# syl051088/DynaAlign

Measured on AMD Instinct MI355X. Metric: sequence-pairs/sec (MinHash k=4 n_hash=500; NW BLOSUM62) at 1/2/4/8 MI355X, higher is better.
Workload: dtype u32

## Files before the change

dynaalign_amd/csrc/minhash_kernels.hip:

```cpp
#include "da_common.hpp"

#include <algorithm>
#include <atomic>
#include <mutex>
#include <vector>
#include <type_traits>

namespace da {
namespace {

__device__ __forceinline__ uint32_t rotl32(uint32_t v, int r) {
  return __builtin_rotateleft32(v, r);
}
__device__ __forceinline__ uint32_t mm3_scramble(uint32_t w) {
  w *= 0xcc9e2d51u;
  w = rotl32(w, 15);
  w *= 0x1b873593u;
  return w;
}
__device__ __forceinline__ uint32_t mm3_mix(uint32_t h, uint32_t kk) {
  h ^= kk;
  return rotl32(h, 13) * 5u + 0xe6546b64u;
}
__device__ __forceinline__ uint32_t mm3_final(uint32_t h, uint32_t len) {
// ... 1442 lines not shown
      uint32_t hi[8] = {0, 0, 0, 0, 0, 0, 0, 0};
      for (int k = 0; k < nhi; ++k) {
        const uint32_t b = blk[rows * W + ((int64_t)k * rows + row) * groups + (col >> 3)];
#pragma unroll
        for (int e = 0; e < 8; ++e) hi[e] |= ((b >> e) & 1u) << (8 + k);
      }
      st[q].x = ((lo.x & 255u) | hi[0]) | ((((lo.x >> 8) & 255u) | hi[1]) << 16);
      st[q].y = (((lo.x >> 16) & 255u) | hi[2]) | (((lo.x >> 24) | hi[3]) << 16);
      st[q].z = ((lo.y & 255u) | hi[4]) | ((((lo.y >> 8) & 255u) | hi[5]) << 16);
      st[q].w = (((lo.y >> 16) & 255u) | hi[6]) | (((lo.y >> 24) | hi[7]) << 16);
    }
  }
  if (!IS_NW)
    for (int e = tid; e < tab_entries; e += 256) tab[e] = (double)e / (double)n_hash;
#pragma unroll
  for (int q = 0; q < 8; ++q) *reinterpret_cast<uint4 *>(er_lds + (row0 + 16 * q) * ER_STRIDE + unit * 16) = st[q];
  __syncthreads();
  auto widen = [&](uint32_t x) -> double {
    if (!IS_NW) return tab_entries ? tab[x] : (double)x / (double)n_hash;
    const uint32_t ln = x & 255u;
    if (ln == 0) return __longlong_as_double(0xFFF8000000000000ULL);
    return (double)(x >> 8) / (double)ln;
  };
  er_store_tile(er_lds, widen, out, ld, I0, J0, tx, ty);
}
static bool finalize_rows_ok(const ShardGeom &geom, const void *d_g, int64_t ld_g, const double *d_out, int64_t ld, bool packed) {
  return geom.tile == 128 && geom.n >= 256 && (ld & 1) == 0 && (reinterpret_cast<uintptr_t>(d_out) & 15) == 0 &&
         (reinterpret_cast<uintptr_t>(d_g) & 15) == 0 && (packed || (ld_g & 7) == 0);
}

template <int FT>
__device__ __forceinline__ void store_tile_u16(const uint16_t (&t)[FT][FT + 2], uint16_t *__restrict__ out, int64_t ld, int n, int i0, int j0) {
  constexpr int RS = 256 / FT;
  const int tx = threadIdx.x & (FT - 1), ty = threadIdx.x / FT;
  const int j = j0 + tx;
  uint16_t *o = out + (int64_t)i0 * ld + j;
  for (int r = ty; r < FT; r += RS) {
    const int i = i0 + r;
    if (i < n && j < n && j >= i) o[(int64_t)r * ld] = t[r][tx];
  }
  const int im = i0 + tx;
  uint16_t *om = out + (int64_t)j0 * ld + im;
  for (int r = ty; r < FT; r += RS) {
    const int jm = j0 + r;
    if (im < n && jm < n && jm > im) om[(int64_t)r * ld] = t[tx][r];
  }
}
template <bool IS_NW, bool U16 = false>
__global__ __launch_bounds__(256) void k_finalize_sharded(const uint16_t *__restrict__ G, int64_t ld_g, ShardGeom geom,
                                                          int n_hash, void *__restrict__ out_v, int64_t ld, int TB,
                                                          int64_t ntiles, int64_t per_xcd, int skip_fast) {
  double *out = static_cast<double *>(out_v);
  constexpr int FT = 64, TABLE = 2048;
  __shared__ uint16_t t[FT][FT + 2];
  __shared__ double ratio[IS_NW ? 1 : TABLE];
  const int n = (int)geom.n;
  const TileId tt = skip_fast ? leftover_tile64(blockIdx.x, n, TB) : decode_tile_xcd(blockIdx.x, per_xcd, ntiles, TB);
  if (!tt.valid) return;
  const int i0 = tt.ti * FT, j0 = tt.tj * FT;
  const int tx = threadIdx.x & 63, ty = threadIdx.x >> 6;
  const bool use_table = !IS_NW && n_hash < TABLE;
  if (use_table)
    for (int c = threadIdx.x; c <= n_hash; c += 256) ratio[c] = (double)c / (double)n_hash;
  auto widen = [&](uint32_t v) -> double {
    if (!IS_NW) return use_table ? ratio[v] : (double)v / (double)n_hash;
    const uint32_t ln = v & 255u;
    if (ln == 0) return __longlong_as_double(0xFFF8000000000000ULL);
    return (double)(v >> 8) / (double)ln;
  };
  const int tile = geom.tile;
  const int tr = i0 / tile;
  const int q = tr / geom.world, owner = tr - q * geom.world;
  const bool front = q <= geom.Q - 1 - q;
  const int64_t lrow0 = (int64_t)owner * geom.rows + (int64_t)(front ? q : geom.Q - 1 - q) * tile + (i0 - tr * tile);
  const int64_t coff = front ? -(int64_t)tr * tile : shard_back(geom.W, geom.n);
  const uint16_t *src = G + lrow0 * ld_g + coff + j0 + tx;
  const int j = j0 + tx;
  for (int r = ty; r < FT; r += 4) {
    const int i = i0 + r;
    if (i < n && j < n && j >= i) t[r][tx] = src[(int64_t)r * ld_g];
  }
  __syncthreads();
  if (U16) store_tile_u16<64>(t, static_cast<uint16_t *>(out_v), ld, n, i0, j0);
  else store_tile_f64<64>(t, widen, out, ld, n, i0, j0);
}

template <bool F64, bool IS_NW, int FT>
__global__ __launch_bounds__(256) void k_expand_unique(const uint16_t *__restrict__ D, int64_t ld_d, const int32_t *__restrict__ uidx,
                                                       int n, int n_hash, void *__restrict__ out_v, int64_t ld, int TB,
                                                       int64_t ntiles, int64_t per_xcd, int skip_fast, TableRows trows) {
  __shared__ uint16_t t[FT][FT + 2];
  __shared__ int32_t ur[FT], uc[FT];
  const TileId tt = skip_fast ? leftover_tile64(blockIdx.x, n, TB) : decode_tile_xcd(blockIdx.x, per_xcd, ntiles, TB);
  if (!tt.valid) return;
  const int i0 = tt.ti * FT, j0 = tt.tj * FT;
  constexpr int RS = 256 / FT;
  const int tx = threadIdx.x & (FT - 1), ty = threadIdx.x / FT;
  for (int q = threadIdx.x; q < 2 * FT; q += 256) {
    if (q < FT) ur[q] = (i0 + q < n) ? uidx[i0 + q] : 0;
    else uc[q - FT] = (j0 + q - FT < n) ? uidx[j0 + q - FT] : 0;
  }
  __syncthreads();
  auto widen = [&](uint32_t v) -> double {
    if (!IS_NW) return (double)v / (double)n_hash;
    const uint32_t ln = v & 255u;
    if (ln == 0) return __longlong_as_double(0xFFF8000000000000ULL);
    return (double)(v >> 8) / (double)ln;
  };
  const int j = j0 + tx;
  const int32_t cj = uc[tx];
  for (int r = ty; r < FT; r += RS) {
    const int i = i0 + r;
    if (i < n && j < n && j >= i) t[r][tx] = D[table_row(ur[r], trows) * ld_d + cj];
  }
  __syncthreads();
  if (F64) {
    store_tile_f64<FT>(t, widen, reinterpret_cast<double *>(out_v), ld, n, i0, j0);
  } else {
    uint16_t *out = reinterpret_cast<uint16_t *>(out_v);
    uint16_t *o = out + (int64_t)i0 * ld + j;
    for (int r = ty; r < FT; r += RS) {
      const int i = i0 + r;
      if (i < n && j < n && j >= i) o[(int64_t)r * ld] = t[r][tx];
    }
    const int im = i0 + tx;
    uint16_t *om = out + (int64_t)j0 * ld + im;
    for (int r = ty; r < FT; r += RS) {
      const int jm = j0 + r;
      if (im < n && jm < n && jm > im) om[(int64_t)r * ld] = t[tx][r];
    }
  }
}

constexpr int GC_THREADS = 1024;
__global__ __launch_bounds__(GC_THREADS) void k_gather_columns(const uint16_t *__restrict__ D, int64_t ld_d, const int32_t *__restrict__ uidx,
                                                               const int32_t *__restrict__ ufirst, int n, int U, uint16_t *__restrict__ F,
                                                               int64_t ld_f, TableRows trows, int from_first_tile, int row_begin) {
  extern __shared__ __attribute__((aligned(16))) uint16_t gc_row[];
  const int units = (int)(ld_d >> 3);
  uint4 pre[8];
#define GC_FETCH(row)                                                                                   \
  {                                                                                                     \
    const uint4 *src_ = reinterpret_cast<const uint4 *>(D + table_row((row), trows) * ld_d);            \
    _Pragma("unroll") for (int q = 0; q < 8; ++q) {                                                     \
      const int u = (int)threadIdx.x + q * GC_THREADS;                                                  \
      pre[q] = u < units ? src_[u] : make_uint4(0, 0, 0, 0);                                            \
    }                                                                                                   \
  }
  int r = row_begin + (int)blockIdx.x;
  if (r < U) GC_FETCH(r)
  const int2 *u2 = reinterpret_cast<const int2 *>(uidx);
  const int j2_end = n >> 1;
  for (; r < U; r += gridDim.x) {
    __syncthreads();
    uint4 *dst = reinterpret_cast<uint4 *>(gc_row);
#pragma unroll
    for (int q = 0; q < 8; ++q) {
      const int u = (int)threadIdx.x + q * GC_THREADS;
      if (u < units) dst[u] = pre[q];
    }
    __syncthreads();
    if (r + (int)gridDim.x < U) GC_FETCH(r + (int)gridDim.x)
    const int j_begin = ((ufirst[r] >> 7) + (from_first_tile ? 0 : 1)) << 7;
    uint32_t *frow = reinterpret_cast<uint32_t *>(F + (int64_t)r * ld_f);
    for (int j2 = (j_begin >> 1) + threadIdx.x; j2 < j2_end; j2 += GC_THREADS) {
      const int2 c = u2[j2];
      __builtin_nontemporal_store((uint32_t)gc_row[c.x] | ((uint32_t)gc_row[c.y] << 16), frow + j2);
    }
    if ((n & 1) && threadIdx.x == 0 && n - 1 >= j_begin) F[(int64_t)r * ld_f + n - 1] = gc_row[uidx[n - 1]];
  }
#undef GC_FETCH
}

template <bool IS_NW>
__global__ __launch_bounds__(256, 4) void k_expand_rows(const uint16_t *__restrict__ F, int64_t ld_f, const int32_t *__restrict__ uidx,
                                                        int n, int n_hash, int tab_stride, int tab_entries, double *__restrict__ out,
                                                        int64_t ld, int T128, int64_t ntiles, int64_t per_xcd, int64_t tile_begin) {
  extern __shared__ __attribute__((aligned(16))) unsigned char er_lds[];
  double *tab = reinterpret_cast<double *>(er_lds + 128 * ER_STRIDE);
  const int64_t L = tile_begin + (int64_t)(blockIdx.x & 7) * per_xcd + (blockIdx.x >> 3);
  if (L >= ntiles || L >= tile_begin + (int64_t)((blockIdx.x & 7) + 1) * per_xcd) return;
  const TileId tt = decode_tile(L, T128, T128, true);
  if (!tt.valid || !expand_fast_takes(tt.ti, tt.tj, n, ld, out)) return;
  const int tid = threadIdx.x, wave = tid >> 6, lane = tid & 63;
  const int tx = ((wave & 1) << 3) + (lane & 7), ty = ((wave >> 1) << 3) + (lane >> 3);
  const int64_t I0 = (int64_t)tt.ti * 128, J0 = (int64_t)tt.tj * 128;
  uint4 st[8];
#pragma unroll
  for (int q = 0; q < 8; ++q) {
    const int row = (tid >> 4) + 16 * q;
    st[q] = *(reinterpret_cast<const uint4 *>(F + (int64_t)uidx[I0 + row] * ld_f + J0) + (tid & 15));
  }
  if (IS_NW) {
    for (int e = tid; e < tab_entries; e += 256) {
      const int mt = e / tab_stride, ln = e - mt * tab_stride;
      tab[e] = ln == 0 ? __longlong_as_double(0xFFF8000000000000ULL) : (double)mt / (double)ln;
    }
  } else {
    for (int e = tid; e < tab_entries; e += 256) tab[e] = (double)e / (double)n_hash;
  }
#pragma unroll
  for (int q = 0; q < 8; ++q)
    *reinterpret_cast<uint4 *>(er_lds + ((tid >> 4) + 16 * q) * ER_STRIDE + (tid & 15) * 16) = st[q];
  __syncthreads();
  auto widen = [&](uint32_t x) -> double {
    if (IS_NW) return tab[(x >> 8) * (uint32_t)tab_stride + (x & 255u)];
    return tab[x];
  };
  er_store_tile(er_lds, widen, out, ld, I0, J0, tx, ty);
}

constexpr int ES_THREADS = 1024, ES_COPIES = 4, ES_BATCH = 16;
__global__ __launch_bounds__(256) void k_es_zero(uint32_t *__restrict__ w, int words) {
  const int i = blockIdx.x * 256 + threadIdx.x;
  if (i < words) w[i] = 0u;
}
__global__ __launch_bounds__(256) void k_es_count(const int32_t *__restrict__ uidx, int n, int U, int Z, uint32_t *__restrict__ cnt) {
  const int i = blockIdx.x * 256 + threadIdx.x;
  if (i < n) atomicAdd(&cnt[(i / Z) * U + uidx[i]], 1u);
}
__device__ __forceinline__ uint64_t es_scan_load(const uint32_t *__restrict__ cnt, int K, int i) {
  const uint32_t c = i < K ? cnt[i] : 0u;
  return (uint64_t)c | ((uint64_t)((c + ES_COPIES - 1) / ES_COPIES) << 32);
}
__global__ __launch_bounds__(1024) void k_es_scan_sums(const uint32_t *__restrict__ cnt, int K, uint64_t *__restrict__ bsum) {
  __shared__ uint64_t wsum[16];
  uint64_t x = es_scan_load(cnt, K, blockIdx.x * 1024 + threadIdx.x);
#pragma unroll
  for (int d = 32; d >= 1; d >>= 1) x += __shfl_xor(x, d, 64);
  if ((threadIdx.x & 63) == 0) wsum[threadIdx.x >> 6] = x;
  __syncthreads();
  if (threadIdx.x == 0) { uint64_t t = 0; for (int w = 0; w < 16; ++w) t += wsum[w]; bsum[blockIdx.x] = t; }
}
__global__ __launch_bounds__(1024) void k_es_scan_offsets(uint64_t *__restrict__ bsum, int nblocks) {
  __shared__ uint64_t wsum[16];
  __shared__ uint64_t carry_s;
  const int tid = threadIdx.x, lane = tid & 63, wave = tid >> 6;
  if (tid == 0) carry_s = 0;
  __syncthreads();
  for (int base = 0; base < nblocks; base += 1024) {
    const int i = base + tid;
    const uint64_t v = i < nblocks ? bsum[i] : 0;
    uint64_t x = v;
#pragma unroll
    for (int d = 1; d < 64; d <<= 1) {
      const uint64_t y = __shfl_up(x, d, 64);
      if (lane >= d) x += y;
    }
    if (lane == 63) wsum[wave] = x;
    __syncthreads();
    uint64_t woff = 0;
    for (int w = 0; w < wave; ++w) woff += wsum[w];
    const uint64_t carry = carry_s;
    if (i < nblocks) bsum[i] = carry + woff + x - v;
    __syncthreads();
    if (tid == 1023) carry_s = carry + woff + x;
    __syncthreads();
  }
  if (tid == 0) bsum[nblocks] = carry_s;
}
__global__ __launch_bounds__(1024) void k_es_scan_apply(const uint32_t *__restrict__ cnt, int K, const uint64_t *__restrict__ bsum,
                                                        uint32_t *__restrict__ cstart, uint32_t *__restrict__ zstart) {
  __shared__ uint64_t wsum[16];
  const int tid = threadIdx.x, lane = tid & 63, wave = tid >> 6;
  const int i = blockIdx.x * 1024 + tid;
  const uint64_t v = es_scan_load(cnt, K, i);
  uint64_t x = v;
#pragma unroll
  for (int d = 1; d < 64; d <<= 1) {
    const uint64_t y = __shfl_up(x, d, 64);
    if (lane >= d) x += y;
  }
  if (lane == 63) wsum[wave] = x;
  __syncthreads();
  uint64_t woff = bsum[blockIdx.x];
  for (int w = 0; w < wave; ++w) woff += wsum[w];
  const uint64_t e = woff + x - v;
  if (i < K) { cstart[i] = (uint32_t)e; zstart[i] = (uint32_t)(e >> 32); }
  if (blockIdx.x == gridDim.x - 1 && tid == 0) { const uint64_t t = bsum[gridDim.x]; cstart[K] = (uint32_t)t; zstart[K] = (uint32_t)(t >> 32); }
}
__global__ __launch_bounds__(256) void k_es_fill(const int32_t *__restrict__ uidx, int n, int U, int Z, int K, const uint32_t *__restrict__ cstart,
                                                 const uint32_t *__restrict__ zstart, uint32_t *__restrict__ cursor, int32_t *__restrict__ cpos,
                                                 int2 *__restrict__ items) {
  const int i = blockIdx.x * 256 + threadIdx.x;
  if (i < n) {
    const int key = (i / Z) * U + uidx[i];
    cpos[cstart[key] + atomicAdd(&cursor[key], 1u)] = i;
  }
  if (i < K) {
    const uint32_t first = zstart[i], cnt = zstart[i + 1] - first;
    for (uint32_t q = 0; q < cnt; ++q) items[first + q] = make_int2(i % U, (int)(q * ES_COPIES));
  }
}
__device__ __forceinline__ double es_ratio(uint32_t c, double dn, double rcp) {
  const double dc = (double)c, q0 = __dmul_rn(dc, rcp), e = __fma_rn(-q0, dn, dc);
  return __fma_rn(e, rcp, q0);
}
__global__ __launch_bounds__(256) void k_es_ratio_check(int n_hash, double *__restrict__ out) {
  const int c = blockIdx.x * 256 + threadIdx.x;
  const double dn = (double)n_hash, rcp = 1.0 / dn;
  if (c <= n_hash) out[c] = es_ratio((uint32_t)c, dn, rcp);
}
enum { ES_U16 = 0, ES_U16_PK = 1, ES_PK = 2 };
#ifdef ES_STEAL_COUNT
__device__ unsigned es_steal[64][ES_ZONES][2];
#endif
template <int FMT, int NQ>
__global__ __launch_bounds__(ES_THREADS, 8)
void k_expand_stream(const uint16_t *__restrict__ D, int64_t ld_d, const int32_t *__restrict__ uidx,
                                                              const uint32_t *__restrict__ cstart, const int32_t *__restrict__ cpos,
                                                              const int2 *__restrict__ items, const uint32_t *__restrict__ zstart, int U, int zones,
                                                              int row_end, int n, int n_hash, double *__restrict__ out, int64_t ld,
                                                              uint32_t *ticket, int max_batch) {
  extern __shared__ __attribute__((aligned(16))) unsigned char es_lds[];
#ifdef ES_PRIO
  __builtin_amdgcn_s_setprio(ES_PRIO);
#endif
  constexpr bool PACKED = FMT != ES_U16;
  uint16_t *row = reinterpret_cast<uint16_t *>(es_lds);
  unsigned char *row_lo = es_lds, *row_hi = row_lo + ld_d;
  const int tid = threadIdx.x;
  const double dn = (double)n_hash, rcp = 1.0 / dn;
  auto count_of = [&](int c) -> uint32_t {
    if (!PACKED) return row[c];
    return (uint32_t)row_lo[c] | ((((uint32_t)row_hi[c >> 3] >> (c & 7)) & 1u) << 8);
  };
  const int64_t row_bytes = FMT == ES_PK ? pk_row_bytes(ld_d) : 2 * ld_d;
  const int units = (int)(row_bytes >> 4);
  uint4 pre[NQ];
#define ES_FETCH(r_)                                                                                    \
  {                                                                                                     \
    const uint4 *src_ = reinterpret_cast<const uint4 *>(reinterpret_cast<const unsigned char *>(D) + (int64_t)(r_) * row_bytes); \
    _Pragma("unroll") for (int q = 0; q < NQ; ++q) {                                                    \
      const int u = tid + q * ES_THREADS;                                                               \
      pre[q] = u < units ? src_[u] : make_uint4(0, 0, 0, 0);                                            \
    }                                                                                                   \
  }
  __shared__ int s_next, s_end, s_zone;
  unsigned home;
  asm volatile("s_getreg_b32 %0, hwreg(HW_REG_XCC_ID)" : "=s"(home));
  home = (home & 7u) % (unsigned)zones;
  const uint32_t home_z0 = zstart[home * U], home_lim = zstart[home * U + row_end] - home_z0,
                 home_all = zstart[home * U + U] - home_z0;
  const uint32_t share = max(1u, gridDim.x / (unsigned)zones);
  auto take = [&]() {
    int tz = -1, tk = 0, te = 0;
    for (int t = 0; t < zones && tz < 0; ++t) {
      const int z = (int)((home + (unsigned)t) % (unsigned)zones);
      const uint32_t z0 = t ? zstart[z * U] : home_z0, lim = t ? zstart[z * U + row_end] - z0 : home_lim,
                     all = t ? zstart[z * U + U] - z0 : home_all;
      uint32_t cur = __hip_atomic_load(&ticket[z], __ATOMIC_RELAXED, __HIP_MEMORY_SCOPE_AGENT);
      while (cur < lim) {
        const uint32_t b = min(min((uint32_t)max_batch, lim - cur), max(1u, (all - cur) / share));
        const uint32_t old = atomicCAS(&ticket[z], cur, cur + b);
#ifdef ES_STEAL_COUNT
        if (old == cur) atomicAdd(&es_steal[min(63, (row_end + 1023) >> 10)][home][t ? 1 : 0], b);
#endif
        if (old == cur) { tz = z; tk = (int)(z0 + cur); te = tk + (int)b; break; }
        cur = old;
      }
    }
    s_zone = tz; s_next = tk; s_end = te;
  };
  if (tid == 0) take();
  __syncthreads();
  int z = __builtin_amdgcn_readfirstlane(s_zone), k = __builtin_amdgcn_readfirstlane(s_next), k_end = __builtin_amdgcn_readfirstlane(s_end);
  int2 it = z >= 0 ? items[k] : make_int2(0, 0);
  if (z >= 0) ES_FETCH(it.x)
  const int2 *u2 = reinterpret_cast<const int2 *>(uidx);
  const int j2_end = n >> 1;
  while (z >= 0) {
    __syncthreads();
    const bool more = k + 1 < k_end;
    if (tid == 0 && !more) take();
    uint4 *dst = reinterpret_cast<uint4 *>(row);
#pragma unroll
    for (int q = 0; q < NQ; ++q) {
      const int u = tid + q * ES_THREADS;
      if (u >= units) continue;
      if (FMT != ES_U16_PK) { dst[u] = pre[q]; continue; }
      const uint4 v = pre[q];
      uint2 lo;
      lo.x = __builtin_amdgcn_perm(v.y, v.x, 0x06040200u);
      lo.y = __builtin_amdgcn_perm(v.w, v.z, 0x06040200u);
      *reinterpret_cast<uint2 *>(row_lo + 8 * u) = lo;
      row_hi[u] = (unsigned char)(((v.x >> 8) & 1u) | ((v.x >> 23) & 2u) | ((v.y >> 6) & 4u) | ((v.y >> 21) & 8u) | ((v.z >> 4) & 16u) |
                                  ((v.z >> 19) & 32u) | ((v.w >> 2) & 64u) | ((v.w >> 17) & 128u));
    }
    __syncthreads();
    const int key = z * U + it.x;
    const uint32_t c0 = cstart[key] + (uint32_t)it.y, c_end = cstart[key + 1];
    const int ncop = (int)min((uint32_t)ES_COPIES, c_end - c0);
    double *orow[ES_COPIES];
#pragma unroll
    for (int q = 0; q < ES_COPIES; ++q) orow[q] = out + (int64_t)cpos[c0 + (uint32_t)min(q, ncop - 1)] * ld;
    const int zn = more ? z : __builtin_amdgcn_readfirstlane(s_zone), kn = more ? k + 1 : __builtin_amdgcn_readfirstlane(s_next);
    if (!more) k_end = __builtin_amdgcn_readfirstlane(s_end);
    int2 itn = make_int2(0, 0);
    if (zn >= 0) { itn = items[kn]; ES_FETCH(itn.x) }
#pragma unroll 4
    for (int j2 = tid; j2 < j2_end; j2 += ES_THREADS) {
      const int2 c = u2[j2];
      const double v0 = es_ratio(count_of(c.x), dn, rcp), v1 = es_ratio(count_of(c.y), dn, rcp);
      nt_store2(orow[0] + 2 * j2, v0, v1);
      if (ncop > 1) nt_store2(orow[1] + 2 * j2, v0, v1);
      if (ncop > 2) nt_store2(orow[2] + 2 * j2, v0, v1);
      if (ncop > 3) nt_store2(orow[3] + 2 * j2, v0, v1);
    }
    if ((n & 1) && tid == 0) {
      const double v = es_ratio(count_of(uidx[n - 1]), dn, rcp);
      for (int q = 0; q < ncop; ++q) orow[q][n - 1] = v;
    }
    it = itn;
    z = zn;
    k = kn;
  }
#undef ES_FETCH
}

bool expand_stream_ok(int64_t n, int64_t U, int n_hash, const void *d_out, int64_t ld) {
  return n >= 2 && n <= 0x7fffffffLL && U >= 1 && U <= 65536 && n_hash >= 1 && n_hash <= 2047 && (ld & 1) == 0 &&
         (reinterpret_cast<uintptr_t>(d_out) & 15) == 0;
}
extern "C" int da_debug_ratio_check(int n_hash, double *d_out, void *stream) {
  if (n_hash < 1 || !d_out) return fail(DA_ERR_BAD_ARG, "ratio check: bad arguments");
  hipLaunchKernelGGL(k_es_ratio_check, dim3((unsigned)(n_hash / 256 + 1)), dim3(256), 0, static_cast<hipStream_t>(stream), n_hash, d_out);
  DA_HIP_TRY(hipGetLastError());
  return DA_OK;
}
#ifdef ES_STEAL_COUNT
extern "C" int da_debug_expand_steals(unsigned *out, int reset) {
  static const unsigned zero[64 * ES_ZONES * 2] = {};
  DA_HIP_TRY(hipDeviceSynchronize());
  if (out) DA_HIP_TRY(hipMemcpyFromSymbol(out, HIP_SYMBOL(es_steal), sizeof(zero)));
  if (reset) DA_HIP_TRY(hipMemcpyToSymbol(HIP_SYMBOL(es_steal), zero, sizeof(zero)));
  return DA_OK;
}
#endif
bool expand_stream_packed(int n_hash) { return n_hash <= 511; }
static int es_zones() { return config().mh_expand_zones == 1 ? 1 : ES_ZONES; }
int expand_stream_zones() { return es_zones(); }
struct EsLists { uint32_t *cnt, *cursor, *ticket, *cstart, *zstart; int32_t *cpos; int2 *items; uint64_t *bsum; int zones, Z, K; size_t bytes; };
static EsLists es_layout(void *d_scratch, int64_t n, int64_t U, int zones) {
  uint32_t *w = static_cast<uint32_t *>(d_scratch);
  EsLists L;
  const int64_t K = (int64_t)zones * U;
  L.zones = zones; L.Z = (int)zone_rows(n, zones); L.K = (int)K;
  L.cnt = w; L.cursor = w + K; L.ticket = w + 2 * K; L.cstart = L.ticket + ES_ZONES; L.zstart = L.cstart + (K + 1);
  L.cpos = reinterpret_cast<int32_t *>(L.zstart + (K + 1));
  L.items = reinterpret_cast<int2 *>((reinterpret_cast<uintptr_t>(L.cpos + n) + 15) & ~(uintptr_t)15);
  L.bsum = reinterpret_cast<uint64_t *>(L.items + (std::min(n, K) + n / ES_COPIES + 2));
  L.bytes = (size_t)(reinterpret_cast<unsigned char *>(L.bsum + (ceil_div(K, 1024) + 1)) - static_cast<unsigned char *>(d_scratch));
  return L;
}
size_t expand_stream_scratch_bytes(int64_t n, int64_t U) {
  return es_layout(nullptr, n, U, ES_ZONES).bytes + 16;
}
static int es_lists(const int32_t *d_uidx, int64_t n, int64_t U, void *d_scratch, int zones, hipStream_t stream) {
  const EsLists L = es_layout(d_scratch, n, U, zones);
  const int zero_words = 2 * L.K + ES_ZONES;
  hipLaunchKernelGGL(k_es_zero, dim3((unsigned)ceil_div(zero_words, 256)), dim3(256), 0, stream, L.cnt, zero_words);
  const unsigned nblk = (unsigned)ceil_div(L.K, 1024);
  hipLaunchKernelGGL(k_es_count, dim3((unsigned)ceil_div(n, 256)), dim3(256), 0, stream, d_uidx, (int)n, (int)U, L.Z, L.cnt);
  hipLaunchKernelGGL(k_es_scan_sums, dim3(nblk), dim3(1024), 0, stream, L.cnt, L.K, L.bsum);
  hipLaunchKernelGGL(k_es_scan_offsets, dim3(1), dim3(1024), 0, stream, L.bsum, (int)nblk);
  hipLaunchKernelGGL(k_es_scan_apply, dim3(nblk), dim3(1024), 0, stream, L.cnt, L.K, L.bsum, L.cstart, L.zstart);
  hipLaunchKernelGGL(k_es_fill, dim3((unsigned)ceil_div(std::max<int64_t>(n, L.K), 256)), dim3(256), 0, stream, d_uidx, (int)n, (int)U, L.Z, L.K,
                     L.cstart, L.zstart, L.cursor, L.cpos, L.items);
  DA_HIP_TRY(hipGetLastError());
  return DA_OK;
}
int launch_expand_stream_lists(const int32_t *d_uidx, int64_t n, int64_t U, void *d_scratch, hipStream_t stream) {
  return es_lists(d_uidx, n, U, d_scratch, es_zones(), stream);
}
extern "C" int da_debug_expand_lists(const int32_t *d_uidx, int64_t n, int64_t U, int zones, void *d_scratch, size_t scratch_bytes, int64_t *offsets_out,
                                     int *zones_out, void *stream) {
  if (zones == 0) zones = es_zones();
  if (n < 1 || n > 0x7fffffffLL || U < 1 || U > 65536 || U > n || (zones != 1 && zones != ES_ZONES) || !offsets_out)
    return fail(DA_ERR_BAD_ARG, "expand lists: bad arguments");
  const EsLists L = es_layout(d_scratch, n, U, zones);
  const unsigned char *b = static_cast<const unsigned char *>(d_scratch);
  offsets_out[0] = reinterpret_cast<const unsigned char *>(L.cstart) - b; offsets_out[1] = reinterpret_cast<const unsigned char *>(L.zstart) - b;
  offsets_out[2] = reinterpret_cast<const unsigned char *>(L.cpos) - b; offsets_out[3] = reinterpret_cast<const unsigned char *>(L.items) - b;
  offsets_out[4] = (int64_t)expand_stream_scratch_bytes(n, U); offsets_out[5] = L.Z;
  if (zones_out) *zones_out = zones;
  if (!d_scratch) return DA_OK;
  if (!d_uidx || scratch_bytes < (size_t)offsets_out[4] || (reinterpret_cast<uintptr_t>(d_scratch) & 15)) return fail(DA_ERR_BAD_ARG, "expand lists: bad scratch");
  return es_lists(d_uidx, n, U, d_scratch, zones, static_cast<hipStream_t>(stream));
}
static int es_launch(const uint16_t *d_D, int64_t ld_d, const int32_t *d_colids, int64_t n_cols, const EsLists &L, int64_t n_rows, int64_t U,
                     int64_t row_end, int n_hash, double *d_out, int64_t ld, hipStream_t stream, bool pk);
int launch_expand_stream_rows(const uint16_t *d_D, int64_t ld_d, const int32_t *d_uidx, int64_t n, int64_t U, int n_hash, double *d_out, int64_t ld,
                              void *d_scratch, int64_t row_end, hipStream_t stream, bool pk) {
  if (!expand_stream_ok(n, U, n_hash, d_out, ld) || (ld_d & (pk ? 127 : 7)) || ld_d > 65536 || (reinterpret_cast<uintptr_t>(d_D) & 15) ||
      (pk && !expand_stream_packed(n_hash)))
    return fail(DA_ERR_UNSUPPORTED, "row expansion: shape not covered");
  if (row_end > U) row_end = U;
  if (row_end <= 0) return DA_OK;
  return es_launch(d_D, ld_d, d_uidx, n, es_layout(d_scratch, n, U, es_zones()), n, U, row_end, n_hash, d_out, ld, stream, pk);
}
static int es_launch(const uint16_t *d_D, int64_t ld_d, const int32_t *d_uidx, int64_t n, const EsLists &L, int64_t n_rows, int64_t U,
                     int64_t row_end, int n_hash, double *d_out, int64_t ld, hipStream_t stream, bool pk) {
  static std::atomic<int> es_cus;
  static std::atomic<uint64_t> es_attr_done;
  int dev = 0;
  DA_HIP_TRY(hipGetDevice(&dev));
  if (!((es_attr_done.load() >> (dev & 63)) & 1u)) {
    hipDeviceProp_t prop;
    DA_HIP_TRY(hipGetDeviceProperties(&prop, dev));
#define DA_ES_ATTR(P, Q) DA_HIP_TRY(hipFuncSetAttribute(reinterpret_cast<const void *>(k_expand_stream<P, Q>), hipFuncAttributeMaxDynamicSharedMemorySize, 65536 * 2))
    DA_ES_ATTR(ES_U16, 2); DA_ES_ATTR(ES_U16, 4); DA_ES_ATTR(ES_U16, 6); DA_ES_ATTR(ES_U16, 8);
    DA_ES_ATTR(ES_U16_PK, 2); DA_ES_ATTR(ES_U16_PK, 4); DA_ES_ATTR(ES_U16_PK, 6); DA_ES_ATTR(ES_U16_PK, 8);
    DA_ES_ATTR(ES_PK, 2); DA_ES_ATTR(ES_PK, 4); DA_ES_ATTR(ES_PK, 6); DA_ES_ATTR(ES_PK, 8);
#undef DA_ES_ATTR
    es_cus.store(prop.multiProcessorCount > 0 ? prop.multiProcessorCount : 256);
    es_attr_done.fetch_or(1ull << (dev & 63));
  }
  const bool packed = pk || expand_stream_packed(n_hash);
  size_t lds = packed ? (size_t)pk_row_bytes(ld_d) : (size_t)ld_d * 2;
  lds = std::max<size_t>(lds, 82 * 1024);
  int64_t grid = (int64_t)es_cus.load();
  grid = std::min<int64_t>(grid, std::min<int64_t>(n_rows, L.K) + n_rows / ES_COPIES + 1);
#define DA_ES(P, Q) hipLaunchKernelGGL((k_expand_stream<P, Q>), dim3((unsigned)grid), dim3(ES_THREADS), lds, stream, d_D, ld_d, d_uidx, L.cstart, L.cpos, L.items, \
                                       L.zstart, (int)U, L.zones, (int)row_end, (int)n, n_hash, d_out, ld, L.ticket, ES_BATCH * ES_ZONES / L.zones)
  const int64_t nq = ceil_div((pk ? pk_row_bytes(ld_d) : 2 * ld_d) >> 4, ES_THREADS);
#define DA_ES_NQ(F) do { if (nq <= 2) DA_ES(F, 2); else if (nq <= 4) DA_ES(F, 4); else if (nq <= 6) DA_ES(F, 6); else DA_ES(F, 8); } while (0)
  if (pk) DA_ES_NQ(ES_PK);
  else if (packed) DA_ES_NQ(ES_U16_PK);
  else DA_ES_NQ(ES_U16);
#undef DA_ES_NQ
#undef DA_ES
  DA_HIP_TRY(hipGetLastError());
  return DA_OK;
}
int launch_expand_stream(const uint16_t *d_D, int64_t ld_d, const int32_t *d_uidx, int64_t n, int64_t U, int n_hash, double *d_out, int64_t ld,
                         void *d_scratch, hipStream_t stream, hipEvent_t after_lists, bool pk) {
  if (!expand_stream_ok(n, U, n_hash, d_out, ld)) return fail(DA_ERR_UNSUPPORTED, "row expansion: shape not covered");
  int rc = launch_expand_stream_lists(d_uidx, n, U, d_scratch, stream);
  if (rc != DA_OK) return rc;
  if (after_lists) DA_HIP_TRY(hipEventRecord(after_lists, stream));
  return launch_expand_stream_rows(d_D, ld_d, d_uidx, n, U, n_hash, d_out, ld, d_scratch, U, stream, pk);
}

bool expand_stream_rect_ok(int64_t m, int64_t n, int64_t U_x, int64_t U_y, int n_hash, const void *d_out, int64_t ld) {
  return m >= 1 && m <= 0x7ffffff0LL && n >= 1 && n <= 0x7ffffff0LL && U_x >= 1 && U_x <= m && U_y >= 1 && U_y <= 65536 && n_hash >= 1 &&
         n_hash <= 2047 && (ld & 1) == 0 && (reinterpret_cast<uintptr_t>(d_out) & 15) == 0;
}
int launch_expand_stream_rect(const uint16_t *d_D, int64_t ld_d, const int32_t *d_uidx_x, int64_t m, int64_t U_x, const int32_t *d_uidx_y, int64_t n,
                              int64_t U_y, int n_hash, double *d_out, int64_t ld, void *d_scratch, hipStream_t stream, hipEvent_t after_lists) {
  if (!expand_stream_rect_ok(m, n, U_x, U_y, n_hash, d_out, ld) || ld_d < U_y || (ld_d & 7) || ld_d > 65536 || (reinterpret_cast<uintptr_t>(d_D) & 15))
    return fail(DA_ERR_UNSUPPORTED, "rectangular row expansion: shape not covered");
  int rc = launch_expand_stream_lists(d_uidx_x, m, U_x, d_scratch, stream);
  if (rc != DA_OK) return rc;
  if (after_lists) DA_HIP_TRY(hipEventRecord(after_lists, stream));
  return es_launch(d_D, ld_d, d_uidx_y, n, es_layout(d_scratch, m, U_x, es_zones()), m, U_x, U_x, n_hash, d_out, ld, stream, false);
}

__global__ __launch_bounds__(256) void k_fill_sig_rows(uint32_t *__restrict__ sig, int64_t ld_sig, int64_t m, int64_t m_pad, int n_hash) {
  const int64_t r = m + blockIdx.x;
  if (r >= m_pad) return;
  const uint32_t *src = sig + ((r - m) % m) * ld_sig;
  for (int h = threadIdx.x; h < n_hash; h += 256) sig[r * ld_sig + h] = src[h];
}
int launch_fill_sig_rows(uint32_t *d_sig, int64_t ld_sig, int64_t m, int64_t m_pad, int n_hash, hipStream_t stream) {
  if (m_pad <= m || m <= 0) return DA_OK;
  hipLaunchKernelGGL(k_fill_sig_rows, dim3((unsigned)(m_pad - m)), dim3(256), 0, stream, d_sig, ld_sig, m, m_pad, n_hash);
  DA_HIP_TRY(hipGetLastError());
  return DA_OK;
}

size_t expand_rows_workspace_bytes(int64_t n, int64_t U, int kind, bool is_nw, int n_hash, int nw_max_len) {
  if (kind != DA_OUT_F64 || n < 256 || U > 65536 || U < 1) return 0;
  if (is_nw ? (nw_max_len < 1 || (int64_t)(nw_max_len + 1) * (2 * nw_max_len + 1) > 2048) : (n_hash < 1 || n_hash + 1 > 2048)) return 0;
  return (size_t)U * (size_t)(ceil_div(n, 8) * 8) * 2;
}

int launch_gather_columns(const uint16_t *d_D, int64_t ld_d, const int32_t *d_uidx, const int32_t *d_ufirst, int64_t n, int64_t U,
                          uint16_t *d_F, int64_t ld_f, bool from_first_tile, hipStream_t stream, int table_world, int64_t table_rows_local,
                          int64_t row_begin, int64_t row_end) {
  if (row_end < 0 || row_end > U) row_end = U;
  if (row_begin < 0) row_begin = 0;
  if (U >= 1 && row_begin >= row_end) return DA_OK;
  if (U < 1 || U > 65536 || (ld_d & 7) || ld_d > 65536 || (reinterpret_cast<uintptr_t>(d_D) & 15) || (ld_f & 1))
    return fail(DA_ERR_UNSUPPORTED, "column gather: at most 65536 unique strings, 16-byte aligned table rows");
  const TableRows trows{table_world, table_rows_local};
  const size_t row_bytes = (size_t)ld_d * 2;
  static std::atomic<int> gc_cus;
  static std::atomic<uint64_t> gc_attr_done;
  int dev = 0;
  DA_HIP_TRY(hipGetDevice(&dev));
  if (!((gc_attr_done.load() >> (dev & 63)) & 1u)) {
    hipDeviceProp_t prop;
    DA_HIP_TRY(hipGetDeviceProperties(&prop, dev));
    DA_HIP_TRY(hipFuncSetAttribute(reinterpret_cast<const void *>(k_gather_columns), hipFuncAttributeMaxDynamicSharedMemorySize, 65536 * 2));
    gc_cus.store(prop.multiProcessorCount > 0 ? prop.multiProcessorCount : 256);
    gc_attr_done.fetch_or(1ull << (dev & 63));
  }
  const int gc_wg = row_bytes <= 40 * 1024 ? 2 : 1;
  const int64_t gc_grid = std::min<int64_t>(row_end - row_begin, (int64_t)gc_cus.load() * gc_wg);
  hipLaunchKernelGGL(k_gather_columns, dim3((unsigned)gc_grid), dim3(GC_THREADS), row_bytes, stream, d_D, ld_d, d_uidx, d_ufirst, (int)n,
                     (int)row_end, d_F, ld_f, trows, from_first_tile ? 1 : 0, (int)row_begin);
  DA_HIP_TRY(hipGetLastError());
  return DA_OK;
}

int launch_expand_rows(const uint16_t *d_F, int64_t ld_f, const int32_t *d_uidx, int64_t n, bool is_nw, int n_hash, int nw_max_len,
                       double *d_out, int64_t ld, int64_t band_begin, int64_t band_end, hipStream_t stream) {
  const int T128 = (int)ceil_div(n, 128);
  if (band_end < 0) band_end = mh_sym_bands(n);
  const int64_t t0 = mh_sym_band_prefix(n, band_begin), t1 = mh_sym_band_prefix(n, band_end);
  if (t1 <= t0) return DA_OK;
  const int64_t px = ceil_div(t1 - t0, 8);
  const int stride = is_nw ? 2 * nw_max_len + 1 : 1;
  const int entries = is_nw ? (nw_max_len + 1) * stride : n_hash + 1;
  const size_t lds = 128 * ER_STRIDE + (size_t)entries * 8;
  if (is_nw) hipLaunchKernelGGL(k_expand_rows<true>, dim3((unsigned)(px * 8)), dim3(256), lds, stream, d_F, ld_f, d_uidx, (int)n, n_hash,
                                stride, entries, d_out, ld, T128, t1, px, t0);
  else hipLaunchKernelGGL(k_expand_rows<false>, dim3((unsigned)(px * 8)), dim3(256), lds, stream, d_F, ld_f, d_uidx, (int)n, n_hash,
                          stride, entries, d_out, ld, T128, t1, px, t0);
  DA_HIP_TRY(hipGetLastError());
  return DA_OK;
}

int launch_expand_unique(const uint16_t *d_D, int64_t ld_d, const int32_t *d_uidx, int64_t n, int kind, bool is_nw, int n_hash,
                         void *d_out, int64_t ld, hipStream_t stream, int nw_max_len, uint16_t *d_F, const int32_t *d_ufirst, int64_t U,
                         hipEvent_t after_gather, hipEvent_t after_rows, int table_world, int64_t table_rows_local, bool only_leftover) {
  const TableRows trows{table_world, table_rows_local};
  if (n <= 0) return DA_OK;
  if (n > 0x7fffffffLL) return fail(DA_ERR_UNSUPPORTED, "expand: matrix too large");
  if (kind != DA_OUT_F64 && kind != DA_OUT_COMPACT) return fail(DA_ERR_BAD_ARG, "expand: bad output kind");
  const int TB = (int)ceil_div(n, 64);
  const int64_t tiles = (int64_t)TB * (TB + 1) / 2;
  if (tiles > 0x7fffffffLL) return fail(DA_ERR_UNSUPPORTED, "matrix too large for one launch");
  const int64_t per_xcd = ceil_div(tiles, 8);
  dim3 grid((unsigned)(per_xcd * 8));
  const bool fast = d_F != nullptr && expand_rows_workspace_bytes(n, U, kind, is_nw, n_hash, nw_max_len) != 0 && (ld & 1) == 0 &&
                    (reinterpret_cast<uintptr_t>(d_out) & 15) == 0;
  if (only_leftover && !fast) return fail(DA_ERR_BAD_ARG, "expand: the streaming passes do not cover this shape");
  if (fast && !only_leftover) {
    const int64_t ld_f = ceil_div(n, 8) * 8;
    int rc_g = launch_gather_columns(d_D, ld_d, d_uidx, d_ufirst, n, U, d_F, ld_f, false, stream, table_world, table_rows_local);
    if (rc_g != DA_OK) return rc_g;
    if (after_gather) DA_HIP_TRY(hipEventRecord(after_gather, stream));
    rc_g = launch_expand_rows(d_F, ld_f, d_uidx, n, is_nw, n_hash, nw_max_len, static_cast<double *>(d_out), ld, 0, -1, stream);
    if (rc_g != DA_OK) return rc_g;
  }
  else if (after_gather) DA_HIP_TRY(hipEventRecord(after_gather, stream));
  if (after_rows) DA_HIP_TRY(hipEventRecord(after_rows, stream));
  const int skip_fast = fast ? 1 : 0;
  if (fast) grid.x = leftover_blocks64(n);
#define DA_EXP(F, W, T) hipLaunchKernelGGL((k_expand_unique<F, W, T>), grid, dim3(256), 0, stream, d_D, ld_d, d_uidx, (int)n, n_hash, d_out, ld, TB, tiles, per_xcd, skip_fast, trows)
  if (kind == DA_OUT_F64) { if (is_nw) DA_EXP(true, true, 64); else DA_EXP(true, false, 64); }
  else { if (is_nw) DA_EXP(false, true, 64); else DA_EXP(false, false, 64); }
#undef DA_EXP
  DA_HIP_TRY(hipGetLastError());
  return DA_OK;
}

int launch_finalize_sharded(const uint16_t *d_g, int64_t ld_g, const ShardGeom &geom, bool is_nw, int n_hash,
                            double *d_out, int64_t ld, hipStream_t stream) {
  if (geom.n <= 0) return DA_OK;
  if (geom.n > 0x7fffffffLL || (geom.tile % 64) != 0) return fail(DA_ERR_UNSUPPORTED, "finalize: unsupported geometry");
  const int TB = (int)ceil_div(geom.n, 64);
  const int64_t tiles = (int64_t)TB * (TB + 1) / 2;
  if (tiles > 0x7fffffffLL) return fail(DA_ERR_UNSUPPORTED, "matrix too large for one launch");
  const int64_t per_xcd = ceil_div(tiles, 8);
  dim3 grid((unsigned)(per_xcd * 8));
  const bool fast = finalize_rows_ok(geom, d_g, ld_g, d_out, ld, false);
  if (fast) {
    const int T128 = (int)ceil_div(geom.n, 128);
    const int64_t t128 = (int64_t)T128 * (T128 + 1) / 2, px = ceil_div(t128, 8);
    const int entries = (!is_nw && n_hash + 1 <= 2048) ? n_hash + 1 : 0;
    const size_t lds = 128 * ER_STRIDE + (size_t)entries * 8;
    if (is_nw) hipLaunchKernelGGL((k_finalize_rows<true, false>), dim3((unsigned)(px * 8)), dim3(256), lds, stream, d_g, ld_g, geom, 0, n_hash, entries,
                                  d_out, ld, T128, t128, px);
    else hipLaunchKernelGGL((k_finalize_rows<false, false>), dim3((unsigned)(px * 8)), dim3(256), lds, stream, d_g, ld_g, geom, 0, n_hash, entries,
                            d_out, ld, T128, t128, px);
    grid.x = leftover_blocks64(geom.n);
  }
  if (is_nw)
    hipLaunchKernelGGL(k_finalize_sharded<true>, grid, dim3(256), 0, stream, d_g, ld_g, geom, n_hash, d_out, ld, TB, tiles, per_xcd, fast ? 1 : 0);
  else
    hipLaunchKernelGGL(k_finalize_sharded<false>, grid, dim3(256), 0, stream, d_g, ld_g, geom, n_hash, d_out, ld, TB, tiles, per_xcd, fast ? 1 : 0);
  DA_HIP_TRY(hipGetLastError());
  return DA_OK;
}

__global__ __launch_bounds__(256) void k_pack_shard(const uint16_t *__restrict__ local, int64_t ld, int64_t rows, int64_t W,
                                                    int nhi, uint8_t *__restrict__ packed) {
  const int64_t groups = W >> 3;
  const int64_t idx = (int64_t)blockIdx.x * 256 + threadIdx.x;
  if (idx >= rows * groups) return;
  const int64_t row = idx / groups, g = idx - row * groups;
  const uint16_t *src = local + row * ld + 8 * g;
  uint32_t v[8];
  if (((ld & 7) == 0) && ((reinterpret_cast<uintptr_t>(local) & 15) == 0)) {
    const uint4 q = *reinterpret_cast<const uint4 *>(src);
    v[0] = q.x & 0xffffu; v[1] = q.x >> 16; v[2] = q.y & 0xffffu; v[3] = q.y >> 16;
    v[4] = q.z & 0xffffu; v[5] = q.z >> 16; v[6] = q.w & 0xffffu; v[7] = q.w >> 16;
  } else {
#pragma unroll
    for (int e = 0; e < 8; ++e) v[e] = src[e];
  }
  uint2 lo;
  lo.x = (v[0] & 255u) | ((v[1] & 255u) << 8) | ((v[2] & 255u) << 16) | ((v[3] & 255u) << 24);
  lo.y = (v[4] & 255u) | ((v[5] & 255u) << 8) | ((v[6] & 255u) << 16) | ((v[7] & 255u) << 24);
  *reinterpret_cast<uint2 *>(packed + row * W + 8 * g) = lo;
  uint8_t *hi = packed + rows * W;
  for (int k = 0; k < nhi; ++k) {
    uint32_t b = 0;
#pragma unroll
    for (int e = 0; e < 8; ++e) b |= ((v[e] >> (8 + k)) & 1u) << e;
    hi[((int64_t)k * rows + row) * groups + g] = (uint8_t)b;
  }
// ... 485 lines not shown
```

Baseline: 347.9 billion.

## Software-pipeline uidx loads and specialize expand-stream store loop per copy count

Restructures the inner expand loop of k_expand_stream. The uidx loads for the next chunk group are now prefetched into registers while the current group is processed, with a sched_barrier and a perm-based pin that keeps the compiler from folding the loads back into the loop. Base addresses are forced into scalar registers via readfirstlane so the stores can use scalar-base addressing, and the store loop is instantiated separately for each copy count (1-4), which removes per-iteration ncop branches. This raises register pressure and code size, and it adds clamped-lane redundant stores in the tail chunk.

```diff
diff --git a/dynaalign_amd/csrc/minhash_kernels.hip b/dynaalign_amd/csrc/minhash_kernels.hip
--- a/dynaalign_amd/csrc/minhash_kernels.hip
+++ b/dynaalign_amd/csrc/minhash_kernels.hip
@@ -1768,6 +1768,14 @@
   if (c <= n_hash) out[c] = es_ratio((uint32_t)c, dn, rcp);
 }
 enum { ES_U16 = 0, ES_U16_PK = 1, ES_PK = 2 };
+constexpr int ES_UNROLL(int nq) { return nq <= 4 ? 4 : 2; }
+typedef int es_int2_t __attribute__((ext_vector_type(2)));
+#define ES_GLOBAL __attribute__((address_space(1)))
+template <class T> __device__ __forceinline__ ES_GLOBAL T *es_scalar_ptr(const void *p) {
+  const uint64_t a = reinterpret_cast<uint64_t>(p);
+  const uint32_t lo = (uint32_t)__builtin_amdgcn_readfirstlane((int)(uint32_t)a), hi = (uint32_t)__builtin_amdgcn_readfirstlane((int)(uint32_t)(a >> 32));
+  return (ES_GLOBAL T *)((uint64_t)lo | ((uint64_t)hi << 32));
+}
 #ifdef ES_STEAL_COUNT
 __device__ unsigned es_steal[64][ES_ZONES][2];
 #endif
@@ -1833,8 +1841,35 @@
   int z = __builtin_amdgcn_readfirstlane(s_zone), k = __builtin_amdgcn_readfirstlane(s_next), k_end = __builtin_amdgcn_readfirstlane(s_end);
   int2 it = z >= 0 ? items[k] : make_int2(0, 0);
   if (z >= 0) ES_FETCH(it.x)
+  constexpr int UNR = ES_UNROLL(NQ);
   const int2 *u2 = reinterpret_cast<const int2 *>(uidx);
   const int j2_end = n >> 1;
+  const int chunks = (j2_end + ES_THREADS - 1) / ES_THREADS;
+  const int whole = j2_end / (UNR * ES_THREADS), rest = chunks - whole * UNR;
+  es_int2_t cur[UNR], cur_rest[1];
+  auto first_of = [&](int chunk) { return min(chunk * ES_THREADS, j2_end - 1); };
+  auto lane_of = [&](int first) { return min((uint32_t)tid, (uint32_t)(j2_end - 1 - first)); };
+  auto ids_of = [&](int chunk, auto &c) {
+#pragma unroll
+    for (int q = 0; q < (int)(sizeof(c) / sizeof(c[0])); ++q) {
+      const int first = first_of(chunk + q);
+      c[q] = es_scalar_ptr<const es_int2_t>(u2 + first)[lane_of(first)];
+    }
+  };
+  auto pin = [&](auto &dst, const auto &src) {
+#pragma unroll
+    for (int q = 0; q < (int)(sizeof(dst) / sizeof(dst[0])); ++q) {
+      dst[q].x = (int)__builtin_amdgcn_perm(0u, (uint32_t)src[q].x, 0x03020100u);
+      dst[q].y = (int)__builtin_amdgcn_perm(0u, (uint32_t)src[q].y, 0x03020100u);
+    }
+  };
+#pragma unroll
+  for (int q = 0; q < UNR; ++q) cur[q] = es_int2_t{0, 0};
+  cur_rest[0] = es_int2_t{0, 0};
+  if (z >= 0 && whole > 0) ids_of(0, cur);
+  if (z >= 0 && rest > 0) ids_of(whole * UNR, cur_rest);
+  pin(cur, cur);
+  pin(cur_rest, cur_rest);
   while (z >= 0) {
     __syncthreads();
     const bool more = k + 1 < k_end;
@@ -1864,18 +1899,42 @@
     if (!more) k_end = __builtin_amdgcn_readfirstlane(s_end);
     int2 itn = make_int2(0, 0);
     if (zn >= 0) { itn = items[kn]; ES_FETCH(itn.x) }
-#pragma unroll 4
-    for (int j2 = tid; j2 < j2_end; j2 += ES_THREADS) {
-      const int2 c = u2[j2];
-      const double v0 = es_ratio(count_of(c.x), dn, rcp), v1 = es_ratio(count_of(c.y), dn, rcp);
-      nt_store2(orow[0] + 2 * j2, v0, v1);
-      if (ncop > 1) nt_store2(orow[1] + 2 * j2, v0, v1);
-      if (ncop > 2) nt_store2(orow[2] + 2 * j2, v0, v1);
-      if (ncop > 3) nt_store2(orow[3] + 2 * j2, v0, v1);
+    auto expand = [&](auto copies) {
+      constexpr int NC = decltype(copies)::value;
+      auto run = [&](auto &ids, int chunk0, int trips) {
+        constexpr int W = (int)(sizeof(ids) / sizeof(ids[0]));
+#pragma unroll 1
+        for (int t = 0; t < trips; ++t) {
+          es_int2_t nxt[W];
+          ids_of(chunk0 + (t + 1 < trips ? t + 1 : 0) * W, nxt);
+#pragma unroll
+          for (int q = 0; q < W; ++q) {
+            const int first = first_of(chunk0 + t * W + q);
+            const uint32_t lane = lane_of(first);
+            const da_double2_t v = {es_ratio(count_of(ids[q].x), dn, rcp), es_ratio(count_of(ids[q].y), dn, rcp)};
+#pragma unroll
+            for (int r = 0; r < NC; ++r)
+              __builtin_nontemporal_store(v, es_scalar_ptr<da_double2_t>(orow[r] + 2 * (int64_t)first) + lane);
+          }
+          __builtin_amdgcn_sched_barrier(0);
+          pin(ids, nxt);
+        }
+      };
+      run(cur, 0, whole);
+      run(cur_rest, whole * UNR, rest);
+    };
+    static_assert(ES_COPIES == 4, "one instance of the store loop per number of copies");
+    switch (ncop) {
+      case 1: expand(std::integral_constant<int, 1>{}); break;
+      case 2: expand(std::integral_constant<int, 2>{}); break;
+      case 3: expand(std::integral_constant<int, 3>{}); break;
+      default: expand(std::integral_constant<int, 4>{}); break;
     }
     if ((n & 1) && tid == 0) {
       const double v = es_ratio(count_of(uidx[n - 1]), dn, rcp);
-      for (int q = 0; q < ncop; ++q) orow[q][n - 1] = v;
+#pragma unroll
+      for (int q = 0; q < ES_COPIES; ++q)
+        if (q < ncop) orow[q][n - 1] = v;
     }
     it = itn;
     z = zn;
```

After: 333.3 billion. 0.958x the previous value.
